# simplify23/MRN

Hardware: AMD Instinct MI355X
Metric: text-line images/sec (fwd+bwd) at 32x256, TRBA+MRN 6 experts (higher is better)
Workload: dtype f32; 1 GPU; MRN loop B: TRBAx6 frozen experts fwd + DM-Router fwd/bwd + clip + Adam, 32x256x4 crops; per_gpu_batch=256, global_batch=256, parallelism=dp1

## Files before the change

### mrn_amd/_lib.py

```python
import ctypes
import os
import re

import torch

_HERE = os.path.dirname(os.path.abspath(__file__))
LIB_PATH = os.environ.get("MRN_LIB_PATH") or os.path.join(_HERE, "csrc", "libmrn_hip.so")
HEADER_PATH = os.path.join(os.path.dirname(_HERE), "include", "mrn_hip.h")
DECODE_HEADER_PATH = os.path.join(os.path.dirname(_HERE), "include", "mrn_decode.h")
ATTN_BEAM_HEADER_PATH = os.path.join(os.path.dirname(_HERE), "include", "mrn_attn_beam.h")
LEXICON_HEADER_PATH = os.path.join(os.path.dirname(_HERE), "include", "mrn_lexicon.h")
ATTN_LEXICON_HEADER_PATH = os.path.join(os.path.dirname(_HERE), "include", "mrn_attn_lexicon.h")

_CTYPES = {
    "int": ctypes.c_int,
    "int64_t": ctypes.c_int64,
    "float": ctypes.c_float,
    "void*": ctypes.c_void_p,
    "float*": ctypes.c_void_p,
    "const float*": ctypes.c_void_p,
    "const int64_t*": ctypes.c_void_p,
    "int64_t*": ctypes.c_void_p,
    "const int*": ctypes.c_void_p,
    "int*": ctypes.c_void_p,
    "const int32_t*": ctypes.c_void_p,
    "int32_t*": ctypes.c_void_p,
    "const void*": ctypes.c_void_p,
    "const void* const*": ctypes.c_void_p,
    "const char*": ctypes.c_char_p,
}


def parse_header(path=HEADER_PATH):
    text = open(path).read()
    text = re.sub(r"/\*.*?\*/", "", text, flags=re.S)
    text = re.sub(r"//[^\n]*", "", text)
    protos = {}
    for m in re.finditer(r"(?m)^\s*((?:const\s+)?\w+\s*\*?)\s*(mrn_\w+)\s*\(([^;{]*?)\)\s*;", text):
        ret = re.sub(r"\s+", " ", m.group(1)).strip().replace(" *", "*")
        name = m.group(2)
        args = m.group(3).strip()
        argtypes, argnames = [], []
        if args and args != "void":
            for a in args.split(","):
                a = re.sub(r"\s+", " ", a).strip()
                mm = re.match(r"(.*?)(\w+)$", a)
                ty = mm.group(1).strip().replace(" *", "*")
                argtypes.append(ty)
                argnames.append(mm.group(2))
        protos[name] = (ret, argtypes, argnames)
    return protos


class _Lib:
    def __init__(self):
        self._dll = None
        self._protos = None

    def load(self):
        if self._dll is not None:
            return self._dll
        if not os.path.exists(LIB_PATH):
            raise RuntimeError(
                f"{LIB_PATH} is missing: build it with `python -m mrn_amd.build` (there is no CPU fallback)")
        dll = ctypes.CDLL(LIB_PATH)
        self._protos = {**parse_header(), **parse_header(DECODE_HEADER_PATH), **parse_header(ATTN_BEAM_HEADER_PATH),
                        **parse_header(LEXICON_HEADER_PATH), **parse_header(ATTN_LEXICON_HEADER_PATH)}
        for name, (ret, argtypes, _) in self._protos.items():
            fn = getattr(dll, name)
            fn.restype = _CTYPES[ret]
            fn.argtypes = [_CTYPES[t] for t in argtypes]
        self._dll = dll
        return dll

    def call(self, name, *args):
        dll = self.load()
        fn = getattr(dll, name)
        rc = fn(*args)
        if fn.restype is ctypes.c_int and rc != 0:
            msg = dll.mrn_last_error().decode()
            raise RuntimeError(f"{name} failed (code {rc}): {msg}")
        return rc


LIB = _Lib()


def call(name, *args):
    return LIB.call(name, *args)
```

### mrn_amd/csrc/conv_first.hip

```cpp
#include "common.hpp"

namespace {

constexpr int PX = 128;
constexpr int PW = PX + 2;
constexpr int CIN = 4;
constexpr int KTOT = 36;

struct ConvFirstParams {
  const float* x;
  const float* w;
  const float* bias;
  const long long* gamma;
  float* y;
  float* stats;
  long x_gstride;
  int G, B, H, W, Cout, act, tiles_w, tiles_h, nblk;
};

template <int NT, bool POOL>
__global__ __launch_bounds__(256) void conv_first_kernel(const ConvFirstParams p) {
  __shared__ __attribute__((aligned(16))) float patch[4 * PW * CIN];
  __shared__ float wl[KTOT * NT * 32];
  __shared__ float red[4 * 2 * NT * 32];
  const int tid = threadIdx.x, lane = tid & 63, wave = tid >> 6;
  const int n31 = lane & 31, kg = lane >> 5;
  int bid = blockIdx.x;
  const int tw = bid % p.tiles_w;
  bid /= p.tiles_w;
  const int th = bid % p.tiles_h;
  bid /= p.tiles_h;
  const int b = bid % p.B;
  const int g = bid / p.B;
  const int x0 = tw * PX, oy0 = th * 2;
  constexpr int Cout = NT * 32;

  const float* xg = p.x + (long)g * p.x_gstride + (long)b * p.H * p.W * CIN;
  for (int i = tid; i < 4 * PW; i += 256) {
    const int r = i / PW, c = i - r * PW;
    const int iy = oy0 - 1 + r, ix = x0 - 1 + c;
    f32x4 v = {0.f, 0.f, 0.f, 0.f};
    if ((unsigned)iy < (unsigned)p.H && (unsigned)ix < (unsigned)p.W) v = *reinterpret_cast<const f32x4*>(xg + ((long)iy * p.W + ix) * CIN);
    *reinterpret_cast<f32x4*>(&patch[i * CIN]) = v;
  }
  const float* wg = p.w + (long)g * Cout * KTOT;
  for (int i = tid; i < KTOT * Cout; i += 256) {
    const int co = i / KTOT, k = i - co * KTOT;
    wl[k * Cout + co] = wg[i];
  }
  __syncthreads();

  f32x16 acc[2][NT];
#pragma unroll
  for (int r = 0; r < 2; ++r)
#pragma unroll
    for (int j = 0; j < NT; ++j)
#pragma unroll
      for (int e = 0; e < 16; ++e) acc[r][j][e] = 0.f;
  const int px = wave * 32 + n31;
#pragma unroll
  for (int s = 0; s < KTOT / 2; ++s) {
    const int tap = s >> 1, ky = tap / 3, kx = tap - ky * 3;
    float wv[NT];
#pragma unroll
    for (int j = 0; j < NT; ++j) wv[j] = wl[(2 * s + kg) * Cout + j * 32 + n31];
#pragma unroll
    for (int r = 0; r < 2; ++r) {
      const float a = patch[((r + ky) * PW + px + kx) * CIN + 2 * (s & 1) + kg];
#pragma unroll
      for (int j = 0; j < NT; ++j) acc[r][j] = __builtin_amdgcn_mfma_f32_32x32x2f32(a, wv[j], acc[r][j], 0, 0, 0);
    }
  }

  const float relu_floor = p.act == 1 ? 0.f : -INFINITY;
  const int Ho = p.H >> 1, Wo = p.W >> 1;
  float* const yg = p.y + (long)g * p.B * (POOL ? Ho * (long)Wo : p.H * (long)p.W) * Cout;
#pragma unroll
  for (int j = 0; j < NT; ++j) {
    const int co = j * 32 + n31;
    const float bv = p.bias ? p.bias[(long)g * Cout + co] : 0.f;
    float sm = 0.f, sq = 0.f;
#pragma unroll
    for (int r = 0; r < 2; ++r) {
      const bool rok = oy0 + r < p.H;
      float* yrow = yg + (((long)b * p.H + oy0 + r) * p.W) * Cout;
#pragma unroll
      for (int e = 0; e < 16; ++e) {
        const int ox = x0 + wave * 32 + (e & 3) + 8 * (e >> 2) + 4 * kg;
        const float v = acc[r][j][e] + bv;
        acc[r][j][e] = v;
        if (rok && ox < p.W) {
          sm += v;
          sq = fmaf(v, v, sq);
          if (!POOL) yrow[(long)ox * Cout + co] = relu_nan(v, relu_floor);
        }
      }
    }
    if (POOL) {
      const float sg = (p.gamma && reinterpret_cast<const float*>(p.gamma[g])[co] < 0.f) ? -1.f : 1.f;
      const int py = oy0 >> 1;
      float* prow = yg + (((long)b * Ho + py) * Wo) * Cout;
#pragma unroll
      for (int e = 0; e < 16; e += 2) {
        const int pxo = (x0 + wave * 32 + (e & 3) + 8 * (e >> 2) + 4 * kg) >> 1;
        const float mx = max_nan(max_nan(acc[0][j][e] * sg, acc[0][j][e + 1] * sg), max_nan(acc[1][j][e] * sg, acc[1][j][e + 1] * sg));
        if (py < Ho && pxo < Wo) prow[(long)pxo * Cout + co] = relu_nan(mx * sg, relu_floor);
      }
    }
    if (p.stats) {
      sm += __shfl_xor(sm, 32);
      sq += __shfl_xor(sq, 32);
      if (kg == 0) {
        red[(wave * 2 + 0) * Cout + co] = sm;
        red[(wave * 2 + 1) * Cout + co] = sq;
      }
    }
  }
  if (p.stats) {
    __syncthreads();
    if (tid < 2 * Cout) {
      const int which = tid / Cout, co = tid - which * Cout;
      float v = 0.f;
#pragma unroll
      for (int w = 0; w < 4; ++w) v += red[(w * 2 + which) * Cout + co];
      const long blk = ((long)b * p.tiles_h + th) * p.tiles_w + tw;
      p.stats[(((long)g * p.nblk + blk) * 2 + which) * Cout + co] = v;
    }
  }
}

}

MRN_EXPORT int64_t mrn_conv3x3_c4_stats_blocks(int B, int H, int W) { return (int64_t)B * ((H + 1) / 2) * ((W + PX - 1) / PX); }

MRN_EXPORT int mrn_conv3x3_c4_grouped_f32(const float* x, const float* w_ohwi, const float* bias, float* y, float* stats, int G,
                                          int64_t x_group_stride, int B, int H, int W, int Cout, int act, int pool,
                                          const void* bn_gamma_ptrs, void* stream) {
  MRN_CHECK_ARG(x && w_ohwi && y && G >= 1 && (Cout == 32 || Cout == 64), "mrn_conv3x3_c4_grouped_f32: bad operands (Cout=%d)", Cout);
  MRN_CHECK_ARG(((uintptr_t)x % 16 == 0) && x_group_stride % 4 == 0 && (uintptr_t)y % 16 == 0 && (!bias || (uintptr_t)bias % 16 == 0),
                "mrn_conv3x3_c4_grouped_f32: input / output / bias must be 16-byte aligned");
  MRN_CHECK_ARG(!pool || (H % 2 == 0 && W % 2 == 0), "mrn_conv3x3_c4_grouped_f32: the pooled form needs even H, W (%d x %d)", H, W);
  if (B == 0 || H == 0 || W == 0) return MRN_OK;
  ConvFirstParams p;
  p.x = x; p.w = w_ohwi; p.bias = bias; p.gamma = (const long long*)bn_gamma_ptrs; p.y = y; p.stats = stats; p.x_gstride = x_group_stride;
  p.G = G; p.B = B; p.H = H; p.W = W; p.Cout = Cout; p.act = act;
  p.tiles_w = (W + PX - 1) / PX;
  p.tiles_h = (H + 1) / 2;
  p.nblk = (int)mrn_conv3x3_c4_stats_blocks(B, H, W);
  const dim3 grid((unsigned)((long)G * B * p.tiles_h * p.tiles_w));
  const hipStream_t st = (hipStream_t)stream;
  if (Cout == 32) {
    if (pool) hipLaunchKernelGGL((conv_first_kernel<1, true>), grid, dim3(256), 0, st, p);
    else hipLaunchKernelGGL((conv_first_kernel<1, false>), grid, dim3(256), 0, st, p);
  } else {
    if (pool) hipLaunchKernelGGL((conv_first_kernel<2, true>), grid, dim3(256), 0, st, p);
    else hipLaunchKernelGGL((conv_first_kernel<2, false>), grid, dim3(256), 0, st, p);
  }
  MRN_LAUNCH_CHECK("conv3x3_c4_grouped");
  return MRN_OK;
}
```

### mrn_amd/csrc/tps.hip

```cpp
#include "common.hpp"

namespace {

constexpr int MAXF = 64;

__global__ __launch_bounds__(256) void tps_sample_kernel(const float* __restrict__ img,
                                                         const float* __restrict__ cprime,
                                                         const float* __restrict__ inv_delta,
                                                         const float* __restrict__ p_hat,
                                                         float* __restrict__ out,
                                                         float* __restrict__ grid_out,
                                                         int H, int W, int Hr, int Wr, int F) {
  __shared__ float T[MAXF][2];
  const int b = blockIdx.y;
  const int F3 = F + 3;
  for (int i = threadIdx.x; i < F3 * 2; i += 256) {
    const int r = i >> 1, d = i & 1;
    float s = 0.f;
    for (int j = 0; j < F; ++j) s = fmaf(inv_delta[r * F3 + j], cprime[((long)b * F + j) * 2 + d], s);
    T[r][d] = s;
  }
  __syncthreads();
  const int n = Hr * Wr;
  const f32x4* im = reinterpret_cast<const f32x4*>(img) + (long)b * H * W;
  for (int p = blockIdx.x * 256 + threadIdx.x; p < n; p += gridDim.x * 256) {
    const float* ph = p_hat + (long)p * F3;
    float gx = 0.f, gy = 0.f;
    for (int j = 0; j < F3; ++j) {
      const float w = ph[j];
      gx = fmaf(w, T[j][0], gx);
      gy = fmaf(w, T[j][1], gy);
    }
    if (grid_out) {
      grid_out[((long)b * n + p) * 2 + 0] = gx;
      grid_out[((long)b * n + p) * 2 + 1] = gy;
    }
    float ix = (gx + 1.f) * 0.5f * (float)(W - 1);
    float iy = (gy + 1.f) * 0.5f * (float)(H - 1);
    ix = fminf(fmaxf(ix, 0.f), (float)(W - 1));
    iy = fminf(fmaxf(iy, 0.f), (float)(H - 1));
    const float fx = floorf(ix), fy = floorf(iy);
    const int x0 = (int)fx, y0 = (int)fy, x1 = x0 + 1, y1 = y0 + 1;
    const float wx1 = ix - fx, wx0 = 1.f - wx1;
    const float wy1 = iy - fy, wy0 = 1.f - wy1;
    const float w_nw = wx0 * wy0, w_ne = wx1 * wy0, w_sw = wx0 * wy1, w_se = wx1 * wy1;
    const bool xin1 = x1 < W, yin1 = y1 < H;
    const f32x4 zero = {0.f, 0.f, 0.f, 0.f};
    const f32x4 nw = im[(long)y0 * W + x0];
    const f32x4 ne = xin1 ? im[(long)y0 * W + x1] : zero;
    const f32x4 sw = yin1 ? im[(long)y1 * W + x0] : zero;
    const f32x4 se = (xin1 && yin1) ? im[(long)y1 * W + x1] : zero;
    f32x4 o;
#pragma unroll
    for (int c = 0; c < 4; ++c) o[c] = nw[c] * w_nw + ne[c] * w_ne + sw[c] * w_sw + se[c] * w_se;
    reinterpret_cast<f32x4*>(out)[(long)b * n + p] = o;
  }
}

}

MRN_EXPORT int mrn_tps_grid_sample_f32(const float* img_nhwc, const float* cprime, const float* inv_delta_c,
                                       const float* p_hat, float* out_nhwc, float* grid_out, int B, int H, int W,
                                       int C, int Hr, int Wr, int F, void* stream) {
  MRN_CHECK_ARG(img_nhwc && cprime && inv_delta_c && p_hat && out_nhwc, "mrn_tps_grid_sample_f32: null operand");
  MRN_CHECK_ARG(C == 4, "mrn_tps_grid_sample_f32: only 4-channel (RGBA) NHWC input is supported, got C=%d", C);
  MRN_CHECK_ARG(F + 3 <= MAXF && F > 0, "mrn_tps_grid_sample_f32: F=%d out of range", F);
  if (B == 0) return MRN_OK;
  dim3 grid(ceil_div(Hr * Wr, 256 * 4), B);
  hipLaunchKernelGGL(tps_sample_kernel, grid, dim3(256), 0, (hipStream_t)stream, img_nhwc, cprime, inv_delta_c, p_hat,
                     out_nhwc, grid_out, H, W, Hr, Wr, F);
  MRN_LAUNCH_CHECK("tps_grid_sample");
  return MRN_OK;
}
```

### mrn_amd/modules/expert_group.py

```python
import os

import torch

from .. import ops
from ._nn import _pair, packed_weight, require_no_grad, to_nhwc
from .geometry import check_call, geometry_supported, unsupported_geometry_message


EVAL_BN_FOLD = os.environ.get("MRN_EVAL_BN_FOLD", "1") != "0"
SVTR_GROUPED_EMBED = os.environ.get("MRN_SVTR_EMBED", "grouped") == "grouped"
TPS_WINO = os.environ.get("MRN_TPS_WINO", "1") == "1"
EVAL_WINO = os.environ.get("MRN_EVAL_WINO", "1") != "0"
SHORTCUT_BN_FOLD = os.environ.get("MRN_SHORTCUT_BN_FOLD", "1") != "0"
RESIDUAL_FROM_F32 = bool(int(os.environ.get("MRN_RESIDUAL_F32", "0")))


def conv_out_rows(H, pool):
    return H if pool is None else ops.conv_out_hw(H, 1, pool[0], pool[1], pool[2])[0]


class Act:

    def __init__(self, shape, f32=None, hl=None, shared=False, wino=None, wino_R=0, affine=None):
        self.shape = tuple(shape)
# ... 417 lines not shown
                x = t if t is not None else x
                qkv = self._linear(name + ".qkv", y_hl, rows, C, [b.mixer.qkv.weight for b in blks],
                                   [b.mixer.qkv.bias for b in blks] if mixer.qkv.bias is not None else None)
                ctx_hl = ops.svtr_attention(qkv.view(G * B, N, 3 * C), mixer.num_heads, mixer.scale, mixer.mask, want_f32=False, want_hl=True,
                                            x3=ops.SVTR_ATTENTION_X3)
            br = self._linear(name + ".proj", ctx_hl, rows, C, [b.mixer.proj.weight for b in blks], [b.mixer.proj.bias for b in blks])
            drop2 = self._drop_scales(blks, B, x.device)
            g2, b2 = self._ln_params(name + ".ln2", [b.norm2 for b in blks])
            x, _, y_hl = ops.add_layernorm_grouped(x, br.view(G * B, N, C), drop1, N, g2, b2, rows, b0.norm2.eps, want_sum=True)
        Ch = blks[0].mlp.fc1.out_features
        if ops.SVTR_FUSED_MLP and (C in (64, 128) or (C == 256 and ops.SVTR_FUSED_MLP256)) and Ch == 4 * C and ops.X3_PRODUCTS == 3:
            fc1s, fc2s = [b.mlp.fc1 for b in blks], [b.mlp.fc2 for b in blks]

            def build():
                w1, s1 = ops.pack_weights_hl32([m.weight.detach().contiguous().view(Ch, 1, 1, C) for m in fc1s])
                perm = ops.mlp_hidden_permutation(Ch, x.device)
                w2, s2 = ops.pack_weights_hl32([m.weight.detach().index_select(1, perm).contiguous().view(C, 1, 1, Ch) for m in fc2s])
                return (w1, s1, torch.stack([m.bias.detach() for m in fc1s]).contiguous(), w2, s2,
                        torch.stack([m.bias.detach() for m in fc2s]).contiguous())
            w1, s1, b1_, w2, s2, b2_ = self._cached(name + ".mlp", [t_ for m in fc1s + fc2s for t_ in (m.weight, m.bias)], build)
            br = ops.svtr_mlp_fused(y_hl, G * rows, rows, G, C, w1, s1, b1_, w2, s2, b2_)
            return x, (br.view(G * B, N, C), drop2)
        hdn_hl = self._linear(name + ".fc1", y_hl, rows, C, [b.mlp.fc1.weight for b in blks], [b.mlp.fc1.bias for b in blks],
                              act=ops.ACT_GELU, hl_only=True)
        br = self._linear(name + ".fc2", hdn_hl, rows, Ch, [b.mlp.fc2.weight for b in blks], [b.mlp.fc2.bias for b in blks])
        return x, (br.view(G * B, N, C), drop2)

    def _svtr(self, image, last_hl=False):
        G = self.G
        nets = [e.FeatureExtraction.ConvNet for e in self.experts]
        n0 = nets[0]
        B = image.shape[0]
        logical = image.permute(0, 3, 1, 2)
        H, W = n0.HW
        N, C = H * W, n0.embed_dim[0]
        x = torch.empty(G * B, N, C, device=image.device, dtype=torch.float32)
        pes = [n.patch_embed for n in nets]
        if SVTR_GROUPED_EMBED and all(p_.proj[1].training for p_ in pes) and C % 32 == 0 and C >= 64:
            a = self.layer(Act((G, B, image.shape[1], image.shape[2], image.shape[3]), image, None, shared=True),
                           [p_.proj[0] for p_ in pes], [p_.proj[1] for p_ in pes], gelu=True)
            tok = self.layer(a, [p_.proj[3] for p_ in pes], [p_.proj[4] for p_ in pes], gelu=True, want_f32=True, want_hl=False).f32
            for g, n in enumerate(nets):
                ops.ew_rows(ops.EW_ADD, tok[g].view(B, N * C), n.pos_embed.view(1, N * C).expand(B, N * C), out=x[g * B:(g + 1) * B].view(B, N * C))
        else:
            for g, n in enumerate(nets):
                tok = n.patch_embed(logical)
                ops.ew_rows(ops.EW_ADD, tok.view(B, N * C), n.pos_embed.view(1, N * C).expand(B, N * C), out=x[g * B:(g + 1) * B].view(B, N * C))
        self._draw_drop_bank(nets, B, image.device)
        for si in range(3):
            blocks = [list(getattr(n, "blocks%d" % (si + 1))) for n in nets]
            pending = None
            for i in range(len(blocks[0])):
                x, pending = self._svtr_block("svtr%d.%d" % (si, i), x, pending, [b[i] for b in blocks], B, N)
            pb, pd = pending if pending is not None else (None, None)
            _, _, hl = ops.add_layernorm_grouped(x, pb, pd, N, want_sum=False, want_f32=False, want_hl=True)
            subs = [getattr(n, "sub_sample%d" % (si + 1)) for n in nets]
            y = self.layer(Act((G, B, H, W, C), None, hl), [s.conv for s in subs], None, relu=False, want_f32=True, want_hl=False)
            _, _, H, W, C = y.shape
            N = H * W
            gm, bt = self._ln_params("svtr_sub%d" % si, [s.norm for s in subs])
            last = si == 2
            _, x, hl = ops.add_layernorm_grouped(y.f32.view(G * B, N, C), None, None, N, gm, bt, B * N, subs[0].norm.eps,
                                                 want_f32=not (last and last_hl), want_hl=last and last_hl)
        return Act((G, B, H, W, C), x.view(G, B, H, W, C) if x is not None else None, hl if last_hl else None)

    def _tps(self, image):
        G = self.G
        B, H, W, C = image.shape
        tps = [e.Transformation for e in self.experts]
        loc = [t.LocalizationNetwork for t in tps]
        pool = ((2, 2), (2, 2), (0, 0))
        x = Act((G, B, H, W, C), image, None, shared=True)
        w2, w3, w4 = (self.wino_for(loc[0].conv[i], [l.conv[i + 1] for l in loc]) if TPS_WINO else 0 for i in (4, 8, 12))
        x = self.layer(x, [l.conv[0] for l in loc], [l.conv[1] for l in loc], pool=pool, want_wino=w2, want_hl=not w2)
        x = self.layer(x, [l.conv[4] for l in loc], [l.conv[5] for l in loc], pool=pool, want_wino=w3, want_hl=not w3)
        x = self.layer(x, [l.conv[8] for l in loc], [l.conv[9] for l in loc], pool=pool, want_wino=w4, want_hl=not w4)
        x = self.layer(x, [l.conv[12] for l in loc], [l.conv[13] for l in loc], want_f32=True, want_hl=False)
        out = torch.empty(G, B, tps[0].I_r_size[0], tps[0].I_r_size[1], C, device=image.device, dtype=torch.float32)
        _, _, Hl, Wl, Cl = x.shape
        v = ops.avgpool_nhwc(x.f32.view(G * B, Hl, Wl, Cl))
        fc1s, fc2s = [l.localization_fc1[0] for l in loc], [l.localization_fc2 for l in loc]
        v = self._batched_linear_f32("loc_fc1", v.view(G, B, Cl), fc1s, act=ops.ACT_RELU)
        cp = self._batched_linear_f32("loc_fc2", v, fc2s).view(G, B, loc[0].F, 2)
        for g, t in enumerate(tps):
            gg = t.GridGenerator
            ops.tps_grid_sample(image, cp[g], gg.inv_delta_C, gg.P_hat, t.I_r_size, out=out[g])
        return Act(tuple(out.shape), out, None)

    def visual_all(self, image, as_act=False):
        stages = self.experts[0].stages
        check_call(stages["Trans"], stages["Feat"], image.shape[0], image.shape[2], image.shape[3])
        img = to_nhwc(image)
        B, H, W, C = img.shape
        self._nbt = []
        self._height_mean = geometry_supported(stages["Feat"], H, W, stages["Trans"])
        if self.experts[0].stages["Trans"] == "TPS":
            x = self._tps(img)
        else:
            x = Act((self.G, B, H, W, C), img, None, shared=True)
        feat = self.experts[0].stages["Feat"]
        if feat == "SVTR":
            for e in self.experts:
                require_no_grad(e.FeatureExtraction.ConvNet, "SVTR")
            x = self._svtr(img, as_act)
        else:
            x = self._resnet(x, as_act) if feat == "ResNet" else self._vgg(x, as_act)
        if self._nbt:
            torch._foreach_add_(self._nbt, 1)
        G, B, Ho, Wo, Cf = x.shape
        if Ho != 1:
            raise NotImplementedError(unsupported_geometry_message(stages["Trans"], stages["Feat"], H, W, Ho))
        return x if as_act else x.f32.view(G, B, Wo, Cf)


class SequenceGroup(_GroupedLinear):

    def __init__(self, extractors):
        self.extractors = list(extractors)
        self.G = len(self.extractors)
        self._cache = {}

    @staticmethod
    def sequence_supported(extractors):
        e0 = extractors[0]
        if len(extractors) < 2 or e0.stages["Seq"] not in ("BiLSTM", "None"):
            return False
        if any(e.stages != e0.stages for e in extractors):
            return False
        return ops.CONV_PRECISION in ("auto", "fp16x3")

    def _bilstm(self, idx, x_hl, rows_shape, K, **dst):
        G = self.G
        B, T = rows_shape
        mods = [e.SequenceModeling[idx] for e in self.extractors]
        H = mods[0].hidden_size
        packed = [m._packed() for m in mods]
        xproj = self._linear("ih%d" % idx, x_hl, B * T, K, [p[0] for p in packed], [p[2] for p in packed])
        w_hh = self._cached("hh%d" % idx, [p[1] for p in packed], lambda: torch.stack([p[1] for p in packed]).contiguous())
        b_hh = self._cached("bhh%d" % idx, [p[3] for p in packed], lambda: torch.stack([p[3] for p in packed]).contiguous())
        if ops.RECURRENT_X3:
            def build():
                packs = [[ops.pack_fragment_major_h(w, H) for w in (m.rnn.weight_hh_l0, m.rnn.weight_hh_l0_reverse)] for m in mods]
                return (torch.stack([torch.stack([d[0] for d in p]) for p in packs]).contiguous(),
                        torch.stack([torch.cat([d[1] for d in p]) for p in packs]).contiguous())
            w_h, w_inv = self._cached("hh16_%d" % idx, [w for m in mods for w in (m.rnn.weight_hh_l0, m.rnn.weight_hh_l0_reverse)], build)
            rec = ops.lstm_layer_x3_grouped(xproj.view(G, B, T, 2 * 4 * H), w_h, w_inv, b_hh, H, 2)
        else:
            rec = ops.lstm_layer_grouped(xproj.view(G, B, T, 2 * 4 * H), w_hh, b_hh, H, 2)
        y = self._linear("lin%d" % idx, ops.split_hl32(rec), B * T, 2 * H, [m.linear.weight for m in mods],
                         [m.linear.bias for m in mods], **dst)
        return y if dst else y.view(G, B, T, -1)

    def sequence(self, visual, out=None, out_row_stride=0, out_group_stride=0):
        _, B, _, T, Cf = visual.shape
        x_hl = visual.hl if visual.hl is not None else ops.split_hl32(visual.f32)
        dst = dict(out=out, out_row_stride=out_row_stride, out_group_stride=out_group_stride) if out is not None else {}
        if self.extractors[0].stages["Seq"] == "BiLSTM":
            y1 = self._bilstm(0, x_hl, (B, T), Cf)
            return self._bilstm(1, ops.split_hl32(y1), (B, T), y1.shape[-1], **dst)
        lins = [e.SequenceModeling[0] for e in self.extractors]
        y = self._linear("seq", x_hl, B * T, Cf, [l.weight for l in lins], [l.bias for l in lins], **dst)
        return y if out is not None else y.view(self.G, B, T, -1)


class HeadsGroup(SequenceGroup):

    def __init__(self, experts):
        self.experts = list(experts)
        super().__init__([e.model for e in self.experts])
# ... 88 lines not shown
```

### mrn_amd/ops.py

```python
import os
import sys
import weakref

import torch

from ._lib import call
from .modules.label_length import ctc_label_length_supported, ctc_uses_long_kernel, unsupported_label_length_message
from .modules.task_count import router_uses_wide_kernels, tasks_supported, unsupported_task_count_message

ACT_NONE, ACT_RELU, ACT_GELU = 0, 1, 2


class KernelTimer:

    def __init__(self, only=None):
        self.spans = []
        self.only = only

    def begin(self, site="other"):
        if self.only is not None and site not in self.only:
            return None
        e = torch.cuda.Event(enable_timing=True)
        e.record()
        return e
# ... 755 lines not shown
            for (kind, p_), val in zip(batched, vals):
                _PREPACKED[(kind, (p_.data_ptr(), p_._version))] = (val, ev, [p_])


MULTI_PACK = os.environ.get("MRN_MULTI_PACK", "1") == "1"
_MULTI_PACK_KINDS = {"lin_fwd_x3": 0, "lin_bwd_x3": 1}
_MULTI_PACK_STATE = {}
MULTI_PACK_STATS = {"calls": 0, "rebuilds": 0, "weights": 0}


def multi_pack_eligible(p, kind):
    if p.dim() != 2 or p.dtype != torch.float32 or not p.is_contiguous() or p.data_ptr() % 16:
        return False
    N, K = p.shape
    return N % 4 == 0 and K % 4 == 0 and (N if _MULTI_PACK_KINDS[kind] else K) % 32 == 0


def multi_pack_linear(entries):
    dev = entries[0][1].device
    sig = tuple((kind, p.data_ptr(), tuple(p.shape)) for kind, p in entries)
    st = _MULTI_PACK_STATE.get(dev)
    if st is None or st["sig"] != sig:
        n = len(entries)
        offs, tiles, total = [], 0, 0
        for kind, p in entries:
            N, K = p.shape
            tr = _MULTI_PACK_KINDS[kind]
            O, I = (K, N) if tr else (N, K)
            offs.append((total, tiles, I // 32, tr))
            tiles += ((O + 31) // 32) * (I // 32)
            total += (N * K * 4 + 255) // 256 * 256
        halves = []
        for _ in range(2):
            out = torch.empty(total, device=dev, dtype=torch.uint8)
            scale = torch.empty(n, 2, device=dev, dtype=torch.float32)
            rows = [[p.data_ptr(), out.data_ptr() + off, scale.data_ptr() + 8 * i, p.shape[0], p.shape[1], tr, t0, ib]
                    for i, ((_, p), (off, t0, ib, tr)) in enumerate(zip(entries, offs))]
            views = [(out[offs[i][0]:offs[i][0] + p.numel() * 4], scale[i:i + 1]) for i, (_, p) in enumerate(entries)]
            halves.append({"desc": torch.tensor(rows, dtype=torch.int64).to(dev), "out": out, "scale": scale, "views": views})
        st = {"sig": sig, "halves": halves, "flip": 0, "amax": torch.zeros(n, device=dev, dtype=torch.int32), "tiles": tiles}
        _MULTI_PACK_STATE[dev] = st
        MULTI_PACK_STATS["rebuilds"] += 1
    half = st["halves"][st["flip"]]
    st["flip"] ^= 1
    call("mrn_multi_pack_linear_hl32", half["desc"].data_ptr(), len(entries), st["tiles"], st["amax"].data_ptr(), FP16_WEIGHT_PEAK, _stream())
    MULTI_PACK_STATS["calls"] += 1
    MULTI_PACK_STATS["weights"] += len(entries)
    return half["views"]


def conv2d_x3_scaled(x, w_ohwi, bias, stride, padding, act=ACT_NONE, want_stats=False, sx=None):
    B, H, W, Cin = x.shape
    Cout, kh, kw, _ = w_ohwi.shape
    x = x.contiguous()
    if sx is None:
        sx = pow2_scale(x, TRAIN_OPERAND_PEAK)
    kind, w_hl, sw = trained_weight_operand(w_ohwi, stride, padding, H)
    if kind == "wino":
        R = WINO_R
        dense = wino_dense(TRAIN_PRODUCTS)
        _, _, v = bn_apply_wino_grouped(x.view(1, B, H, W, Cin), None, None, R, relu=False, prescale=sx, dense=dense)
        y, stats = conv2d_x3_wino(v, 1, False, B, H, W, Cin, w_hl, sw, Cout, R, bias=bias, act=act, want_stats=want_stats, x_scale=sx, dense=dense)
        return y[0], stats
    y, stats = conv2d_x3(split_hl32(x, sx), 1, False, B, H, W, Cin, w_hl, sw, Cout, (kh, kw), stride, padding, bias=bias, act=act,
                         want_stats=want_stats, x_scale=sx, products=TRAIN_PRODUCTS)
    return y[0], stats


def conv2d_x3_frozen(x, packed, bias, stride, padding, act=ACT_NONE, want_stats=False):
    B, H, W, Cin = x.shape
    Cout, kh, kw, _ = packed.shape
    x = x.contiguous()
    wino = WINO_R in (2, 4) and X3_PRODUCTS == 3 and wino_eligible((kh, kw), stride, padding, Cin, Cout)
    w_hl, sw = packed.x3_operand(wino)
    if wino:
        _, _, v = bn_apply_wino_grouped(x.view(1, B, H, W, Cin), None, None, WINO_R, relu=False)
        y, stats = conv2d_x3_wino(v, 1, False, B, H, W, Cin, w_hl, sw, Cout, WINO_R, bias=bias, act=act, want_stats=want_stats)
        return y[0], stats
    y, stats = conv2d_x3(split_hl32(x), 1, False, B, H, W, Cin, w_hl, sw, Cout, (kh, kw), stride, padding, bias=bias, act=act,
                         want_stats=want_stats, products=X3_PRODUCTS)
    return y[0], stats


def conv3x3_c4_grouped(x, weights, bias=None, act=ACT_NONE, want_stats=False, out=None, pool=False, gamma_ptrs=None):
    _chk(x, weights, bias)
    G, Cout = weights.shape[0], weights.shape[1]
    shared = x.dim() == 4
    B, H, W, C = x.shape[-4:]
    assert C == 4 and x.is_contiguous() and weights.is_contiguous() and tuple(weights.shape[2:]) == (3, 3, 4)
    Ho, Wo = (H // 2, W // 2) if pool else (H, W)
    y = out if out is not None else torch.empty(G, B, Ho, Wo, Cout, device=x.device, dtype=torch.float32)
    stats = None
    if want_stats:
        nblk = call("mrn_conv3x3_c4_stats_blocks", B, H, W)
        stats = torch.empty(G, nblk, 2, Cout, device=x.device, dtype=torch.float32)
    t0 = CONV_TIMER.begin() if CONV_TIMER is not None else None
    call("mrn_conv3x3_c4_grouped_f32", _p(x), _p(weights), _p(bias), _p(y), _p(stats), G, 0 if shared else B * H * W * 4, B, H, W,
         Cout, act, int(bool(pool)), _p(gamma_ptrs), _stream())
    if t0 is not None:
        CONV_TIMER.end(t0, 2.0 * G * B * H * W * Cout * 36, ("f32mfma/" if pool else "hbm/") + "conv_first_kernel<%d%s>" % (Cout // 32, ", true" if pool else ""),
                       4.0 * ((1 if shared else G) * B * H * W * 4 + G * B * Ho * Wo * Cout))
    return y, stats


PATCH_CONV = os.environ.get("MRN_PATCH_CONV", "1") == "1"


def patch_conv_supported(ksize, stride, padding, Cin, Cout):
    return (PATCH_CONV and tuple(ksize) == (3, 3) and tuple(stride) == (1, 1) and tuple(padding) == (1, 1)
            and bool(call("mrn_conv3x3_patch_supported", Cin, Cout)))


def conv3x3_patch_x3(x_hl, G, shared_input, B, H, W, Cin, w_hl, w_scale, Cout, bias=None, act=ACT_NONE, want_stats=False, pool=False,
                     gamma_ptrs=None, out=None):
    dev = x_hl.device
    Ho, Wo = (H // 2, W // 2) if pool else (H, W)
    y = out if out is not None else torch.empty(G, B, Ho, Wo, Cout, device=dev, dtype=torch.float32)
    stats = None
    if want_stats:
        stats = torch.empty(G, call("mrn_conv3x3_patch_stats_blocks", G, B, H, W, Cin), 2, Cout, device=dev, dtype=torch.float32)
    timed = CONV_TIMER is not None
    t0 = CONV_TIMER.begin() if timed else None
    one = X3_PRODUCTS == 1
    call("mrn_conv3x3_patch_x1_hl32" if one else "mrn_conv3x3_patch_x3_hl32", _p(x_hl), _p(w_hl), _p(w_scale), _p(bias), _p(gamma_ptrs), _p(y),
         _p(stats), G, 0 if shared_input else B * H * W * Cin * 4, B, H, W, Cin, Cout, act, int(bool(pool)), _stream())
    if timed:
        nbytes = 4.0 * ((1 if shared_input else G) * B * H * W * Cin + G * Cout * 9 * Cin + G * B * Ho * Wo * Cout)
        kind = ("fp16" if one else "fp16x3") + "/patch%d" % Cin + ("pool" if pool else "")
        if TIMER_SHAPES:
            kind += "|G%d B%d %dx%d %d->%d k3x3 s11" % (G, B, H, W, Cin, Cout)
        CONV_TIMER.end(t0, 2.0 * G * B * H * W * Cout * 9 * Cin, kind, nbytes)
    return y, stats


_FINALIZE_TICKETS = {}


def _finalize_tickets(device, slots):
    key = _dev_stream()
    t = _FINALIZE_TICKETS.get(key)
    if t is None or t.numel() < slots:
        t = torch.zeros(max(slots, 1024), device=device, dtype=torch.int32)
        _FINALIZE_TICKETS[key] = t
    return t


def bn_finalize_grouped(stats, G, C, count, ptr_table, momentum, eps):
    scale = torch.empty(G, C, device=stats.device, dtype=torch.float32)
    shift = torch.empty(G, C, device=stats.device, dtype=torch.float32)
    nblk = stats.numel() // (2 * C * G)
    Z = call("mrn_bn_finalize_grouped_chunks", nblk)
    ws = tk = None
    if Z > 1:
        slots = G * ((C + 31) // 32)
        ws = torch.empty(slots * Z * 64, device=stats.device, dtype=torch.float64)
        tk = _finalize_tickets(stats.device, slots)
    call("mrn_bn_finalize_grouped_f32", _p(stats), G, nblk, C, count, _p(ptr_table), float(momentum), float(eps), _p(scale),
         _p(shift), _p(ws), _p(tk), _stream())
    return scale, shift


def bn_eval_affine_grouped(ptr_table, G, C, eps):
    scale = torch.empty(G, C, device=ptr_table.device, dtype=torch.float32)
    shift = torch.empty(G, C, device=ptr_table.device, dtype=torch.float32)
    call("mrn_bn_eval_affine_grouped_f32", _p(ptr_table), G, C, float(eps), _p(scale), _p(shift), _stream())
    return scale, shift
# ... 77 lines not shown
_SCALE_CACHE = {}
FUSED_AMAX = os.environ.get("MRN_FUSED_AMAX", "1") == "1"


def cached_scale(x):
    e = _SCALE_CACHE.pop(id(x), None)
    return e[1] if (e is not None and e[0]() is x) else None


def clear_scale_cache():
    _SCALE_CACHE.clear()


def scale_shift_act(x, scale, shift, relu=True, residual=None, out=None, range_target=None, pos_mask=None):
    C = x.shape[-1]
    rows = x.numel() // C
    if out is None:
        out = x
    ws = _amax_ws() if (range_target is not None and FUSED_AMAX) else None
    call("mrn_scale_shift_act_f32", _p(x), _p(residual), _p(out), _p(scale), _p(shift), rows, C, int(relu), ws, _p(pos_mask), _stream())
    if ws is not None:
        sc = torch.empty(2, device=x.device, dtype=torch.float32)
        call("mrn_pow2_finalize_f32", float(range_target), _p(sc), ws, _stream())
        if len(_SCALE_CACHE) > 256:
            clear_scale_cache()
        _SCALE_CACHE[id(out)] = (weakref.ref(out), sc)
    return out


def maxpool_nhwc(x, kernel, stride, padding=(0, 0), scale=None, shift=None, relu=False):
    B, H, W, C = x.shape
    Ho, Wo = conv_out_hw(H, W, kernel, stride, padding)
    y = torch.empty(B, Ho, Wo, C, device=x.device, dtype=torch.float32)
    call("mrn_maxpool_nhwc_f32", _p(x), _p(y), _p(scale), _p(shift), int(relu), B, H, W, C, kernel[0], kernel[1],
         stride[0], stride[1], padding[0], padding[1], _stream())
    return y


def avgpool_nhwc(x, scale=None, shift=None, relu=False):
    B, H, W, C = x.shape
    y = torch.empty(B, C, device=x.device, dtype=torch.float32)
    call("mrn_avgpool_nhwc_f32", _p(x), _p(y), _p(scale), _p(shift), int(relu), B, H * W, C, _stream())
    return y


def height_mean_grouped(x, scale=None, shift=None, relu=False, want_f32=True, want_hl=False):
    _chk(x, scale, shift)
    G, B, H, W, C = x.shape
    assert x.is_contiguous()
    out = torch.empty(G, B, W, C, device=x.device, dtype=torch.float32) if want_f32 else None
    out_hl = torch.empty(G * B * W * C * 4, device=x.device, dtype=torch.uint8) if want_hl else None
    t0 = CONV_TIMER.begin("hmean") if CONV_TIMER is not None else None
    call("mrn_height_mean_grouped_f32", _p(x), _p(scale), _p(shift), int(bool(relu)), _p(out), _p(out_hl), G, B, H, W, C, _stream())
    if t0 is not None:
        CONV_TIMER.end(t0, 0.0, "hbm/height_mean_grouped", 4.0 * x.numel() + 4.0 * G * B * W * C * (int(want_f32) + int(want_hl)))
    return out, out_hl


def height_mean(x):
    B, H, W, C = x.shape
    return height_mean_grouped(x.contiguous().view(1, B, H, W, C))[0].view(B, W, C)


def height_mean_bwd(dy, H):
    _chk(dy)
    B, W, C = dy.shape
    dx = torch.empty(B, H, W, C, device=dy.device, dtype=torch.float32)
    call("mrn_height_mean_bwd_f32", _p(dy.contiguous()), _p(dx), B, H, W, C, _stream())
    return dx


def tps_grid_sample(img_nhwc, cprime, inv_delta_c, p_hat, out_hw, want_grid=False, out=None):
    _chk(img_nhwc, cprime, inv_delta_c, p_hat)
    B, H, W, C = img_nhwc.shape
    Hr, Wr = out_hw
    F = cprime.shape[1]
    if out is None:
        out = torch.empty(B, Hr, Wr, C, device=img_nhwc.device, dtype=torch.float32)
    assert out.is_contiguous() and out.numel() == B * Hr * Wr * C
    grid = torch.empty(B, Hr * Wr, 2, device=img_nhwc.device, dtype=torch.float32) if want_grid else None
    call("mrn_tps_grid_sample_f32", _p(img_nhwc), _p(cprime.contiguous()), _p(inv_delta_c), _p(p_hat), _p(out),
         _p(grid), B, H, W, C, Hr, Wr, F, _stream())
    return (out, grid) if want_grid else out


def pack_fragment_major(w, hidden=256):
    G = w.shape[0] // hidden
    K = w.shape[1]
    assert w.shape[0] == G * hidden and hidden % 16 == 0 and K % 16 == 0
    v = w.reshape(G, hidden // 16, 16, K // 16, 4, 4)
    return v.permute(1, 0, 3, 4, 2, 5).contiguous()


def lstm_layer(xproj, w_hh, b_hh, hidden, ndir, save=False):
    _chk(xproj, w_hh, b_hh)
    B, T, _ = xproj.shape
    out = torch.empty(B, T, ndir * hidden, device=xproj.device, dtype=torch.float32)
    gates = cseq = None
    if save:
        gates = torch.empty(B, T, ndir, 4 * hidden, device=xproj.device, dtype=torch.float32)
        cseq = torch.empty(B, T, ndir, hidden, device=xproj.device, dtype=torch.float32)
    call("mrn_lstm_layer_fwd_f32", _p(xproj), _p(w_hh), _p(b_hh), _p(out), _p(gates), _p(cseq), B, T, hidden, ndir, _stream())
    return (out, gates, cseq) if save else out


TRAIN_LSTM_X3 = os.environ.get("MRN_TRAIN_LSTM_X3", "1") == "1"


def lstm_layer_x3_save(xproj, w_hh_h, w_inv, b_hh, hidden, ndir):
    _chk(xproj, b_hh)
    B, T, _ = xproj.shape
    assert xproj.is_contiguous() and w_hh_h.is_contiguous() and w_inv.is_contiguous()
    out = torch.empty(B, T, ndir * hidden, device=xproj.device, dtype=torch.float32)
    gates = torch.empty(B, T, ndir, 4 * hidden, device=xproj.device, dtype=torch.float32)
    cseq = torch.empty(B, T, ndir, hidden, device=xproj.device, dtype=torch.float32)
    call("mrn_lstm_layer_fwd_x3_save", _p(xproj), _p(w_hh_h), _p(w_inv), _p(b_hh), _p(out), _p(gates), _p(cseq), B, T, hidden, ndir, _stream())
    return out, gates, cseq


def _ptrs(ts):
    import ctypes
    return (ctypes.c_void_p * len(ts))(*[t.data_ptr() for t in ts])


def _x3_call(stem, grouped, w_inv, head, tail):
    if w_inv is None:
        return call(f"mrn_{stem}_grouped_f32" if grouped else f"mrn_{stem}_f32", *head, *tail)
    return call(f"mrn_{stem}_x3_grouped" if grouped else f"mrn_{stem}_x3", *head, _ptrs(w_inv) if grouped else _p(w_inv), *tail)


def pack_fragment_major_h(w, hidden=256):
    G = w.shape[0] // hidden
    K = w.shape[1]
    assert w.shape[0] == G * hidden and hidden % 16 == 0 and K % 32 == 0
    sc = pow2_scale(w.contiguous())
    v = (w * sc[0]).reshape(G, hidden // 16, 16, K // 32, 4, 8).permute(1, 0, 3, 4, 2, 5)
    hi = v.half()
    lo = (v - hi.float()).half()
    return torch.stack([hi, lo], dim=5).contiguous(), sc[1:2].clone()


def lstm_layer_x3_grouped(xproj, w_hh_h, w_inv, b_hh, hidden, ndir):
    _chk(xproj, b_hh)
    G, B, T, _ = xproj.shape
    assert xproj.is_contiguous() and w_hh_h.is_contiguous() and w_inv.is_contiguous() and b_hh.is_contiguous()
    out = torch.empty(G, B, T, ndir * hidden, device=xproj.device, dtype=torch.float32)
    call("mrn_lstm_layer_fwd_x3_grouped", _ptrs(xproj), _ptrs(w_hh_h), _ptrs(w_inv), _ptrs(b_hh), _ptrs(out), G, B, T, hidden, ndir, _stream())
    return out




def lstm_layer_grouped(xproj, w_hh, b_hh, hidden, ndir):
    _chk(xproj, w_hh, b_hh)
    G, B, T, _ = xproj.shape
    assert xproj.is_contiguous() and w_hh.is_contiguous() and b_hh.is_contiguous()
    out = torch.empty(G, B, T, ndir * hidden, device=xproj.device, dtype=torch.float32)
    call("mrn_lstm_layer_fwd_grouped_f32", _ptrs(xproj), _ptrs(w_hh), _ptrs(b_hh), _ptrs(out), G, B, T, hidden, ndir, _stream())
    return out


def attn_decoder_grouped(Hb, Hproj, eproj, w_h2h, b_h2h, w_score, w_ih, w_hh, b_hh, hidden, w_inv=None):
    _chk(Hb, Hproj, eproj)
    G, B, T, D = Hb.shape
    S = eproj.shape[2]
    assert Hb.is_contiguous() and Hproj.is_contiguous() and eproj.is_contiguous()
# ... 1288 lines not shown
```

Baseline: 3178 images/s.

## Add persistent double-buffered first-conv kernel and optional grouped TPS sampling

Adds a persistent version of the first 3x3 C=4 conv. Each workgroup walks a contiguous range of tiles, keeps its weights in registers, and double-buffers the input patch in LDS so the next tile's global loads overlap the current tile's MFMA work. Statistics are flushed one tile late and the MFMA/LDS schedule is interleaved by hand. It is on by default and selected through an env var or a new select API. A grouped TPS grid-sample kernel that launches all experts in one call is also added, but it sits behind MRN_TPS_GROUPED (off by default). The persistent kernel costs more register and LDS pressure, and the boundary tiles take a slower staged epilogue.

```diff
diff --git a/include/mrn_first_conv.h b/include/mrn_first_conv.h
--- /dev/null
+++ b/include/mrn_first_conv.h
@@ -0,0 +1,18 @@
+#ifndef MRN_FIRST_CONV_H
+#define MRN_FIRST_CONV_H
+#include <stdint.h>
+
+#ifdef __cplusplus
+extern "C" {
+#endif
+
+int mrn_conv3x3_c4_select(int mode, int max_workgroups);
+
+int mrn_tps_grid_sample_grouped_f32(const float* img_nhwc, const float* cprime, const void* grid_tables, float* out_nhwc, int G,
+                                    int64_t cprime_group_stride, int64_t out_group_stride, int B, int H, int W, int C, int Hr,
+                                    int Wr, int F, void* stream);
+
+#ifdef __cplusplus
+}
+#endif
+#endif
diff --git a/mrn_amd/_lib.py b/mrn_amd/_lib.py
--- a/mrn_amd/_lib.py
+++ b/mrn_amd/_lib.py
@@ -11,6 +11,7 @@
 ATTN_BEAM_HEADER_PATH = os.path.join(os.path.dirname(_HERE), "include", "mrn_attn_beam.h")
 LEXICON_HEADER_PATH = os.path.join(os.path.dirname(_HERE), "include", "mrn_lexicon.h")
 ATTN_LEXICON_HEADER_PATH = os.path.join(os.path.dirname(_HERE), "include", "mrn_attn_lexicon.h")
+FIRST_CONV_HEADER_PATH = os.path.join(os.path.dirname(_HERE), "include", "mrn_first_conv.h")
 
 _CTYPES = {
     "int": ctypes.c_int,
@@ -65,7 +66,8 @@
                 f"{LIB_PATH} is missing: build it with `python -m mrn_amd.build` (there is no CPU fallback)")
         dll = ctypes.CDLL(LIB_PATH)
         self._protos = {**parse_header(), **parse_header(DECODE_HEADER_PATH), **parse_header(ATTN_BEAM_HEADER_PATH),
-                        **parse_header(LEXICON_HEADER_PATH), **parse_header(ATTN_LEXICON_HEADER_PATH)}
+                        **parse_header(LEXICON_HEADER_PATH), **parse_header(ATTN_LEXICON_HEADER_PATH),
+                        **parse_header(FIRST_CONV_HEADER_PATH)}
         for name, (ret, argtypes, _) in self._protos.items():
             fn = getattr(dll, name)
             fn.restype = _CTYPES[ret]
diff --git a/mrn_amd/csrc/conv_first.hip b/mrn_amd/csrc/conv_first.hip
--- a/mrn_amd/csrc/conv_first.hip
+++ b/mrn_amd/csrc/conv_first.hip
@@ -1,4 +1,5 @@
 #include "common.hpp"
+#include <type_traits>
 
 namespace {
 
@@ -129,6 +130,266 @@
   }
 }
 
+constexpr int PWP = 132;
+constexpr int PRE = (4 * PW + 255) / 256;
+
+struct FirstTile {
+  int tw, th, b, g;
+};
+
+template <int NT, bool POOL>
+__global__ __launch_bounds__(256, 4) void conv_first_persistent_kernel(const ConvFirstParams p, const long tiles) {
+  constexpr int Cout = NT * 32;
+  __shared__ float patch[2][4 * CIN * PWP];
+  __shared__ float red[2][4 * 2 * Cout];
+  __shared__ float stage[16 * 256];
+  const int tid = threadIdx.x, lane = tid & 63, wave = tid >> 6;
+  const int n31 = lane & 31, kg = lane >> 5;
+  const long t0 = tiles * blockIdx.x / gridDim.x, t1 = tiles * (blockIdx.x + 1) / gridDim.x;
+  if (t0 >= t1) return;
+
+  FirstTile cur;
+  {
+    long q = t0;
+    cur.tw = (int)(q % p.tiles_w);
+    q /= p.tiles_w;
+    cur.th = (int)(q % p.tiles_h);
+    q /= p.tiles_h;
+    cur.b = (int)(q % p.B);
+    cur.g = (int)(q / p.B);
+  }
+  auto fetch = [&](const FirstTile& c, f32x4 (&v)[PRE]) {
+    int ft = tid;
+    asm volatile("" : "+v"(ft));
+    const int iy = c.th * 2 - 1 + (ft >> 6), ix0 = c.tw * PX - 1 + (ft & 63);
+    const bool rok = (unsigned)iy < (unsigned)p.H;
+    const int iyc = min(max(iy, 0), p.H - 1);
+    const float* xr = p.x + (long)c.g * p.x_gstride + ((long)c.b * p.H + iyc) * p.W * CIN;
+    int ok = 0;
+#pragma unroll
+    for (int k = 0; k < PRE; ++k) {
+      const int ix = ix0 + 64 * k;
+      v[k] = *reinterpret_cast<const f32x4*>(xr + (long)min(max(ix, 0), p.W - 1) * CIN);
+      ok |= (rok && (unsigned)ix < (unsigned)p.W) ? 1 << k : 0;
+    }
+    return ok;
+  };
+  auto stash = [&](float* buf, const f32x4 (&v)[PRE], int ok) {
+    int ft = tid;
+    asm volatile("" : "+v"(ft));
+    float* row = buf + (ft >> 6) * CIN * PWP + (ft & 63);
+#pragma unroll
+    for (int k = 0; k < PRE; ++k) {
+      if ((ft & 63) + 64 * k < PW) {
+#pragma unroll
+        for (int c = 0; c < CIN; ++c) row[c * PWP + 64 * k] = (ok >> k & 1) ? v[k][c] : 0.f;
+      }
+    }
+  };
+  auto flush = [&](const float* rd, long slot) {
+    if (tid < 2 * Cout) {
+      float v = 0.f;
+#pragma unroll
+      for (int w = 0; w < 4; ++w) v += rd[w * 2 * Cout + tid];
+      float* sp = p.stats + slot * 2 * Cout;
+      int ft = tid;
+      asm volatile("" : "+v"(ft));
+      sp[ft] = v;
+    }
+  };
+
+  f32x4 pre[PRE];
+  int preok = fetch(cur, pre);
+  stash(patch[0], pre, preok);
+
+  float wreg[KTOT / 2][NT], bv[NT], sg[NT];
+  int gw = -1;
+  long pend = -1;
+  int par = 0;
+  const float relu_floor = p.act == 1 ? 0.f : -INFINITY;
+  const int Ho = p.H >> 1, Wo = p.W >> 1;
+  const int px = wave * 32 + n31;
+
+  for (long t = t0;; ++t) {
+    const int g = cur.g, b = cur.b, x0 = cur.tw * PX, oy0 = cur.th * 2;
+    if (t < t1 && g != gw) {
+      gw = g;
+      const float* wg = p.w + (long)g * Cout * KTOT;
+#pragma unroll
+      for (int j = 0; j < NT; ++j) {
+        const int co = j * 32 + n31;
+#pragma unroll
+        for (int s = 0; s < KTOT / 2; ++s) wreg[s][j] = wg[co * KTOT + 2 * s + kg];
+        bv[j] = p.bias ? p.bias[(long)g * Cout + co] : 0.f;
+        sg[j] = (POOL && p.gamma && reinterpret_cast<const float*>(p.gamma[g])[co] < 0.f) ? -1.f : 1.f;
+      }
+#pragma unroll
+      for (int j = 0; j < NT; ++j)
+#pragma unroll
+        for (int s = 0; s < KTOT / 2; ++s) asm volatile("" : "+v"(wreg[s][j]));
+    }
+    FirstTile nxt = cur;
+    if (++nxt.tw == p.tiles_w) {
+      nxt.tw = 0;
+      if (++nxt.th == p.tiles_h) {
+        nxt.th = 0;
+        if (++nxt.b == p.B) {
+          nxt.b = 0;
+          ++nxt.g;
+        }
+      }
+    }
+    const bool more = t + 1 < t1;
+    __syncthreads();
+    if (p.stats && pend >= 0) flush(red[par ^ 1], pend);
+    if (t == t1) break;
+    __builtin_amdgcn_sched_barrier(0);
+
+    const float* pt = patch[par] + px;
+    float* const yg = p.y + (long)g * p.B * (POOL ? Ho * (long)Wo : p.H * (long)p.W) * Cout;
+    float* const rw = red[par];
+    const int oxl = x0 + wave * 32 + 4 * kg;
+    const bool inner = x0 + PX <= p.W && oy0 + 2 <= p.H;
+#pragma unroll
+    for (int j = 0; j < NT; ++j) {
+      if (j == NT - 1 && more) preok = fetch(nxt, pre);
+      f32x16 acc[2];
+#pragma unroll
+      for (int r = 0; r < 2; ++r)
+#pragma unroll
+        for (int e = 0; e < 16; ++e) acc[r][e] = 0.f;
+#pragma unroll
+      for (int s = 0; s < KTOT / 2; ++s) {
+        const int tap = s >> 1, ky = tap / 3, kx = tap - ky * 3;
+#pragma unroll
+        for (int r = 0; r < 2; ++r) {
+          const float a = pt[((r + ky) * CIN + 2 * (s & 1) + kg) * PWP + kx];
+          acc[r] = __builtin_amdgcn_mfma_f32_32x32x2f32(a, wreg[s][j], acc[r], 0, 0, 0);
+        }
+      }
+      __builtin_amdgcn_sched_group_barrier(0x100, 4, 0);
+#pragma unroll
+      for (int s = 0; s < KTOT / 2 - 2; ++s) {
+        __builtin_amdgcn_sched_group_barrier(0x008, 2, 0);
+        __builtin_amdgcn_sched_group_barrier(0x100, 2, 0);
+      }
+      __builtin_amdgcn_sched_group_barrier(0x008, 4, 0);
+      __builtin_amdgcn_sched_barrier(0);
+      if (j == NT - 1 && more) stash(patch[par ^ 1], pre, preok);
+      __builtin_amdgcn_sched_barrier(0);
+
+      const int co = j * 32 + n31;
+      auto epilogue = [&](auto inner_t) {
+        constexpr bool INNER = decltype(inner_t)::value;
+        float sm = 0.f, sq = 0.f;
+        const int py = oy0 >> 1;
+        float* prow = yg + (((long)b * Ho + py) * Wo + (oxl >> 1)) * Cout + co;
+        if constexpr (INNER) {
+#pragma unroll
+          for (int r = 0; r < 2; ++r) {
+            float* yrow = yg + (((long)b * p.H + oy0 + r) * p.W + oxl) * Cout + co;
+#pragma unroll
+            for (int e = 0; e < 16; ++e) {
+              const float v = acc[r][e] + bv[j];
+              acc[r][e] = v;
+              sm += v;
+              sq = fmaf(v, v, sq);
+              if (!POOL) yrow[((e & 3) + 8 * (e >> 2)) * Cout] = relu_nan(v, relu_floor);
+            }
+          }
+          if (POOL) {
+#pragma unroll
+            for (int e = 0; e < 16; e += 2) {
+              const float mx = max_nan(max_nan(acc[0][e] * sg[j], acc[0][e + 1] * sg[j]), max_nan(acc[1][e] * sg[j], acc[1][e + 1] * sg[j]));
+              prow[(((e & 3) + 8 * (e >> 2)) >> 1) * Cout] = relu_nan(mx * sg[j], relu_floor);
+            }
+          }
+        } else {
+#pragma unroll
+          for (int r = 0; r < 2; ++r) {
+            const bool rok = oy0 + r < p.H;
+            float* yrow = yg + (((long)b * p.H + oy0 + r) * p.W + oxl) * Cout + co;
+#pragma unroll
+            for (int e = 0; e < 16; ++e) stage[e * 256 + tid] = acc[r][e];
+#pragma nounroll
+            for (int e = 0; e < 16; ++e) {
+              const int dx = (e & 3) + 8 * (e >> 2);
+              const float v = stage[e * 256 + tid] + bv[j];
+              if (rok && oxl + dx < p.W) {
+                sm += v;
+                sq = fmaf(v, v, sq);
+                if (!POOL) yrow[dx * Cout] = relu_nan(v, relu_floor);
+              }
+            }
+          }
+          if (POOL) {
+#pragma unroll
+            for (int e = 0; e < 16; e += 2) {
+              const int dx = ((e & 3) + 8 * (e >> 2)) >> 1;
+              const float mx = max_nan(max_nan((acc[0][e] + bv[j]) * sg[j], (acc[0][e + 1] + bv[j]) * sg[j]),
+                                       max_nan((acc[1][e] + bv[j]) * sg[j], (acc[1][e + 1] + bv[j]) * sg[j]));
+              if (py < Ho && (oxl >> 1) + dx < Wo) prow[dx * Cout] = relu_nan(mx * sg[j], relu_floor);
+            }
+          }
+        }
+        if (p.stats) {
+          sm += __shfl_xor(sm, 32);
+          sq += __shfl_xor(sq, 32);
+          if (kg == 0) {
+            rw[(wave * 2 + 0) * Cout + co] = sm;
+            rw[(wave * 2 + 1) * Cout + co] = sq;
+          }
+        }
+      };
+      if (inner) epilogue(std::true_type{});
+      else epilogue(std::false_type{});
+      __builtin_amdgcn_sched_barrier(0);
+    }
+    pend = (long)g * p.nblk + ((long)b * p.tiles_h + cur.th) * p.tiles_w + cur.tw;
+    par ^= 1;
+    cur = nxt;
+  }
+}
+
+template <int NT, bool POOL>
+int persistent_slots() {
+  static int slots = 0;
+  if (slots == 0) {
+    int dev = 0, per = 0;
+    hipDeviceProp_t prop;
+    int cus = 256;
+    if (hipGetDevice(&dev) == hipSuccess && hipGetDeviceProperties(&prop, dev) == hipSuccess && prop.multiProcessorCount > 0)
+      cus = prop.multiProcessorCount;
+    if (hipOccupancyMaxActiveBlocksPerMultiprocessor(&per, conv_first_persistent_kernel<NT, POOL>, 256, 0) != hipSuccess || per < 1) per = 4;
+    slots = cus * per;
+  }
+  return slots;
+}
+
+template <int NT, bool POOL>
+void launch_persistent(const ConvFirstParams& p, int max_wgs, hipStream_t st) {
+  const long tiles = (long)p.G * p.B * p.tiles_h * p.tiles_w;
+  long wgs = max_wgs > 0 ? max_wgs : persistent_slots<NT, POOL>();
+  if (wgs > tiles) wgs = tiles;
+  hipLaunchKernelGGL((conv_first_persistent_kernel<NT, POOL>), dim3((unsigned)wgs), dim3(256), 0, st, p, tiles);
+}
+
+int g_first_mode = -1;
+int g_first_max_wgs = 0;
+
+bool first_persistent() {
+  static const bool env_off = getenv("MRN_FIRST_CONV_PERSISTENT") && atoi(getenv("MRN_FIRST_CONV_PERSISTENT")) == 0;
+  return g_first_mode >= 0 ? g_first_mode == 1 : !env_off;
+}
+
+}
+
+MRN_EXPORT int mrn_conv3x3_c4_select(int mode, int max_workgroups) {
+  MRN_CHECK_ARG(mode >= -1 && mode <= 1 && max_workgroups >= 0, "mrn_conv3x3_c4_select: mode %d / max_workgroups %d out of range", mode,
+                max_workgroups);
+  g_first_mode = mode;
+  g_first_max_wgs = max_workgroups;
+  return MRN_OK;
 }
 
 MRN_EXPORT int64_t mrn_conv3x3_c4_stats_blocks(int B, int H, int W) { return (int64_t)B * ((H + 1) / 2) * ((W + PX - 1) / PX); }
@@ -149,7 +410,15 @@
   p.nblk = (int)mrn_conv3x3_c4_stats_blocks(B, H, W);
   const dim3 grid((unsigned)((long)G * B * p.tiles_h * p.tiles_w));
   const hipStream_t st = (hipStream_t)stream;
-  if (Cout == 32) {
+  if (first_persistent()) {
+    if (Cout == 32) {
+      if (pool) launch_persistent<1, true>(p, g_first_max_wgs, st);
+      else launch_persistent<1, false>(p, g_first_max_wgs, st);
+    } else {
+      if (pool) launch_persistent<2, true>(p, g_first_max_wgs, st);
+      else launch_persistent<2, false>(p, g_first_max_wgs, st);
+    }
+  } else if (Cout == 32) {
     if (pool) hipLaunchKernelGGL((conv_first_kernel<1, true>), grid, dim3(256), 0, st, p);
     else hipLaunchKernelGGL((conv_first_kernel<1, false>), grid, dim3(256), 0, st, p);
   } else {
diff --git a/mrn_amd/csrc/tps.hip b/mrn_amd/csrc/tps.hip
--- a/mrn_amd/csrc/tps.hip
+++ b/mrn_amd/csrc/tps.hip
@@ -4,15 +4,10 @@
 
 constexpr int MAXF = 64;
 
-__global__ __launch_bounds__(256) void tps_sample_kernel(const float* __restrict__ img,
-                                                         const float* __restrict__ cprime,
-                                                         const float* __restrict__ inv_delta,
-                                                         const float* __restrict__ p_hat,
-                                                         float* __restrict__ out,
-                                                         float* __restrict__ grid_out,
-                                                         int H, int W, int Hr, int Wr, int F) {
-  __shared__ float T[MAXF][2];
-  const int b = blockIdx.y;
+__device__ __forceinline__ void tps_sample_image(float (*T)[2], const float* __restrict__ img, const float* __restrict__ cprime,
+                                                 const float* __restrict__ inv_delta, const float* __restrict__ p_hat,
+                                                 float* __restrict__ out, float* __restrict__ grid_out, int b, int bx, int nbx, int H, int W,
+                                                 int Hr, int Wr, int F) {
   const int F3 = F + 3;
   for (int i = threadIdx.x; i < F3 * 2; i += 256) {
     const int r = i >> 1, d = i & 1;
@@ -23,7 +18,7 @@
   __syncthreads();
   const int n = Hr * Wr;
   const f32x4* im = reinterpret_cast<const f32x4*>(img) + (long)b * H * W;
-  for (int p = blockIdx.x * 256 + threadIdx.x; p < n; p += gridDim.x * 256) {
+  for (int p = bx * 256 + threadIdx.x; p < n; p += nbx * 256) {
     const float* ph = p_hat + (long)p * F3;
     float gx = 0.f, gy = 0.f;
     for (int j = 0; j < F3; ++j) {
@@ -57,6 +52,29 @@
   }
 }
 
+__global__ __launch_bounds__(256) void tps_sample_kernel(const float* __restrict__ img,
+                                                         const float* __restrict__ cprime,
+                                                         const float* __restrict__ inv_delta,
+                                                         const float* __restrict__ p_hat,
+                                                         float* __restrict__ out,
+                                                         float* __restrict__ grid_out,
+                                                         int H, int W, int Hr, int Wr, int F) {
+  __shared__ float T[MAXF][2];
+  tps_sample_image(T, img, cprime, inv_delta, p_hat, out, grid_out, blockIdx.y, blockIdx.x, gridDim.x, H, W, Hr, Wr, F);
+}
+
+__global__ __launch_bounds__(256) void tps_sample_grouped_kernel(const float* __restrict__ img,
+                                                                 const float* __restrict__ cprime,
+                                                                 const long long* __restrict__ tables,
+                                                                 float* __restrict__ out,
+                                                                 long cprime_gstride, long out_gstride, int H, int W, int Hr, int Wr, int F) {
+  __shared__ float T[MAXF][2];
+  const int g = blockIdx.z, G = gridDim.z;
+  tps_sample_image(T, img, cprime + g * cprime_gstride, reinterpret_cast<const float*>(tables[g]),
+                   reinterpret_cast<const float*>(tables[G + g]), out + g * out_gstride, nullptr, blockIdx.y, blockIdx.x, gridDim.x, H, W, Hr,
+                   Wr, F);
+}
+
 }
 
 MRN_EXPORT int mrn_tps_grid_sample_f32(const float* img_nhwc, const float* cprime, const float* inv_delta_c,
@@ -72,3 +90,20 @@
   MRN_LAUNCH_CHECK("tps_grid_sample");
   return MRN_OK;
 }
+
+MRN_EXPORT int mrn_tps_grid_sample_grouped_f32(const float* img_nhwc, const float* cprime, const void* grid_tables, float* out_nhwc,
+                                               int G, int64_t cprime_group_stride, int64_t out_group_stride, int B, int H, int W,
+                                               int C, int Hr, int Wr, int F, void* stream) {
+  MRN_CHECK_ARG(img_nhwc && cprime && grid_tables && out_nhwc, "mrn_tps_grid_sample_grouped_f32: null operand");
+  MRN_CHECK_ARG(C == 4, "mrn_tps_grid_sample_grouped_f32: only 4-channel (RGBA) NHWC input is supported, got C=%d", C);
+  MRN_CHECK_ARG(F + 3 <= MAXF && F > 0, "mrn_tps_grid_sample_grouped_f32: F=%d out of range", F);
+  MRN_CHECK_ARG(G >= 1 && G <= 65535 && B <= 65535, "mrn_tps_grid_sample_grouped_f32: G=%d, B=%d out of range", G, B);
+  MRN_CHECK_ARG(out_group_stride % 4 == 0 && (uintptr_t)out_nhwc % 16 == 0 && (uintptr_t)img_nhwc % 16 == 0,
+                "mrn_tps_grid_sample_grouped_f32: images must be 16-byte aligned");
+  if (B == 0) return MRN_OK;
+  dim3 grid(ceil_div(Hr * Wr, 256 * 4), B, G);
+  hipLaunchKernelGGL(tps_sample_grouped_kernel, grid, dim3(256), 0, (hipStream_t)stream, img_nhwc, cprime, (const long long*)grid_tables,
+                     out_nhwc, (long)cprime_group_stride, (long)out_group_stride, H, W, Hr, Wr, F);
+  MRN_LAUNCH_CHECK("tps_grid_sample_grouped");
+  return MRN_OK;
+}
diff --git a/mrn_amd/modules/expert_group.py b/mrn_amd/modules/expert_group.py
--- a/mrn_amd/modules/expert_group.py
+++ b/mrn_amd/modules/expert_group.py
@@ -523,9 +523,19 @@
         fc1s, fc2s = [l.localization_fc1[0] for l in loc], [l.localization_fc2 for l in loc]
         v = self._batched_linear_f32("loc_fc1", v.view(G, B, Cl), fc1s, act=ops.ACT_RELU)
         cp = self._batched_linear_f32("loc_fc2", v, fc2s).view(G, B, loc[0].F, 2)
-        for g, t in enumerate(tps):
-            gg = t.GridGenerator
-            ops.tps_grid_sample(image, cp[g], gg.inv_delta_C, gg.P_hat, t.I_r_size, out=out[g])
+        gens = [t.GridGenerator for t in tps]
+        if ops.TPS_GROUPED and all(tuple(t.I_r_size) == tuple(tps[0].I_r_size) and gg.P_hat.shape == gens[0].P_hat.shape
+                                   for t, gg in zip(tps, gens)):
+            key = tuple(t.data_ptr() for gg in gens for t in (gg.inv_delta_C, gg.P_hat))
+            got = self._bncache.get(("tps", id(gens[0])))
+            if got is None or got[0] != key:
+                got = (key, ops.tps_grid_tables([gg.inv_delta_C for gg in gens], [gg.P_hat for gg in gens]))
+                self._bncache[("tps", id(gens[0]))] = got
+            ops.tps_grid_sample_grouped(image, cp.contiguous(), got[1], tps[0].I_r_size, out=out)
+        else:
+            for g, t in enumerate(tps):
+                gg = t.GridGenerator
+                ops.tps_grid_sample(image, cp[g], gg.inv_delta_C, gg.P_hat, t.I_r_size, out=out[g])
         return Act(tuple(out.shape), out, None)
 
     def visual_all(self, image, as_act=False):
diff --git a/mrn_amd/ops.py b/mrn_amd/ops.py
--- a/mrn_amd/ops.py
+++ b/mrn_amd/ops.py
@@ -861,6 +861,10 @@
     return y[0], stats
 
 
+def first_conv_select(mode=-1, max_workgroups=0):
+    call("mrn_conv3x3_c4_select", int(mode), int(max_workgroups))
+
+
 def conv3x3_c4_grouped(x, weights, bias=None, act=ACT_NONE, want_stats=False, out=None, pool=False, gamma_ptrs=None):
     _chk(x, weights, bias)
     G, Cout = weights.shape[0], weights.shape[1]
@@ -1104,6 +1108,29 @@
     call("mrn_tps_grid_sample_f32", _p(img_nhwc), _p(cprime.contiguous()), _p(inv_delta_c), _p(p_hat), _p(out),
          _p(grid), B, H, W, C, Hr, Wr, F, _stream())
     return (out, grid) if want_grid else out
+
+
+TPS_GROUPED = os.environ.get("MRN_TPS_GROUPED", "0") == "1"
+
+
+def tps_grid_tables(inv_delta_cs, p_hats):
+    _chk(*inv_delta_cs, *p_hats)
+    return torch.tensor([[t.data_ptr() for t in inv_delta_cs], [t.data_ptr() for t in p_hats]], dtype=torch.int64,
+                        device=inv_delta_cs[0].device)
+
+
+def tps_grid_sample_grouped(img_nhwc, cprime, tables, out_hw, out=None):
+    _chk(img_nhwc, cprime)
+    B, H, W, C = img_nhwc.shape
+    G, F = cprime.shape[0], cprime.shape[2]
+    Hr, Wr = out_hw
+    assert cprime.is_contiguous() and tuple(cprime.shape) == (G, B, F, 2) and tuple(tables.shape) == (2, G) and img_nhwc.is_contiguous()
+    if out is None:
+        out = torch.empty(G, B, Hr, Wr, C, device=img_nhwc.device, dtype=torch.float32)
+    assert out.is_contiguous() and out.numel() == G * B * Hr * Wr * C
+    call("mrn_tps_grid_sample_grouped_f32", _p(img_nhwc), _p(cprime), _p(tables), _p(out), G, B * F * 2, B * Hr * Wr * C, B, H, W, C,
+         Hr, Wr, F, _stream())
+    return out
 
 
 def pack_fragment_major(w, hidden=256):
```

After: 3204 images/s, median of 6. Within noise of the previous version (+0.8%).
